# vsergeev/luaradio

Hardware: AMD Instinct MI355X
Metric: MSamples/s per block (128-tap complex FIR headline) + WBFM chain end-to-end (higher is better)
Workload: dtype f32

## Files before the change

### luaradio_amd/csrc/kernels_channelizer.h

```cpp
#pragma once
#include "common.h"
#include "kernels_fir.h"

#ifndef LRHIP_CHAN_EXP
#define LRHIP_CHAN_EXP 0
#endif

namespace lrhip {

#ifndef LRHIP_CHAN_INTERLEAVE
#define LRHIP_CHAN_INTERLEAVE 1
#endif
#ifndef LRHIP_CHAN_RT
#define LRHIP_CHAN_RT 1
#endif
#ifndef LRHIP_CHAN_KSLAB
#define LRHIP_CHAN_KSLAB 32
#endif
constexpr int CHAN_RT = LRHIP_CHAN_RT;
constexpr int CHAN_MT = 64 * CHAN_RT;
constexpr int CHAN_KSLAB = LRHIP_CHAN_KSLAB;

template <int NCT>
__global__ __launch_bounds__(256, CHAN_RT == 1 ? 2 : 1) void channelizer_kernel(const float *__restrict__ hist, const float *__restrict__ x,
                                                             const float *__restrict__ W, float *__restrict__ y,
                                                             int M, long n, long nframes, long first)
{
    constexpr int K2 = 16 * NCT;
    constexpr int K = K2 / 2;
    constexpr int DROW = K2 + 2;
    constexpr int WROW = K2 + 16;
    extern __shared__ __attribute__((aligned(16))) float lds[];
    const int tid = threadIdx.x, lane = tid & 63, wave = tid >> 6;
    const int col = lane & 15, kq = lane >> 4;
    const long f0 = (long)blockIdx.x * CHAN_MT;
    const int nsamp = (CHAN_MT - 1) * K + M;
    const int nflt = 2 * nsamp;
    float *ldsD = lds;
    const int dsize = ((nflt + 2 * (nflt / K2) + 2 + 3) / 4) * 4;
    float *ldsW = lds + dsize;

    const long p0 = first + f0 * K;
    const long xlo = p0 - (M - 1);
    if (xlo >= 0 && xlo + nsamp <= n && ((reinterpret_cast<uintptr_t>(x + 2 * xlo) & 15) == 0)) {
        const float4 *src = reinterpret_cast<const float4 *>(x + 2 * xlo);
        for (int i4 = tid; i4 < nflt / 4; i4 += 256) {
            float4 v = src[i4];
            int a = 4 * i4, p = a + 2 * (a / K2);
            *reinterpret_cast<float2 *>(ldsD + p) = make_float2(v.x, v.y);
            *reinterpret_cast<float2 *>(ldsD + p + 2) = make_float2(v.z, v.w);
        }
        for (int a = (nflt / 4) * 4 + tid; a < nflt; a += 256) ldsD[a + 2 * (a / K2)] = x[2 * xlo + a];
    } else {
        for (int r = tid; r < nsamp; r += 256) {
            int a = 2 * r, p = a + 2 * (a / K2);
            ldsD[p] = stream_at<2>(hist, x, p0 + r, 0, M, n);
            ldsD[p + 1] = stream_at<2>(hist, x, p0 + r, 1, M, n);
        }
    }

    constexpr int SLAB_F4 = CHAN_KSLAB * K2 / 4;
    constexpr int UW = (SLAB_F4 + 255) / 256;
    const float4 *W4 = reinterpret_cast<const float4 *>(W);
    static_assert(UW <= 8, "W slab prefetch: at most 8 float4 per thread");
    float4 w0, w1, w2, w3, w4, w5, w6, w7;
#define LR_CHAN_FOR8(OP) OP(0) OP(1) OP(2) OP(3) OP(4) OP(5) OP(6) OP(7)
#define LR_CHAN_LOAD(U)                                                                          \
    if (U < UW) {                                                                                \
        int i4 = tid + U * 256;                                                                  \
        w##U = W4[wbase + (i4 < SLAB_F4 ? i4 : SLAB_F4 - 1)];                                    \
    }
#define LR_CHAN_PUT(U)                                                                           \
    if (U < UW) {                                                                                \
        int i4 = tid + U * 256;                                                                  \
        if (i4 < SLAB_F4) *reinterpret_cast<float4 *>(wdst + ((4 * i4) / K2) * WROW + (4 * i4) % K2) = w##U; \
    }
    {
        const size_t wbase = 0;
        float *wdst = ldsW;
        LR_CHAN_FOR8(LR_CHAN_LOAD)
        LR_CHAN_FOR8(LR_CHAN_PUT)
    }
    __syncthreads();

    f32x4 acc[CHAN_RT][NCT];
#pragma unroll
    for (int r = 0; r < CHAN_RT; r++)
#pragma unroll
        for (int c = 0; c < NCT; c++) acc[r][c] = (f32x4){0.f, 0.f, 0.f, 0.f};
    const float *abase = ldsD + DROW * (wave * 16 * CHAN_RT + col) + kq;
    const int nslabs = 2 * M / CHAN_KSLAB;
    for (int s = 0; s < nslabs; s++) {
        const float *wcur = ldsW + (s & 1) * (CHAN_KSLAB * WROW);
#if LRHIP_CHAN_EXP == 1
        const bool more = false;
#else
        const bool more = s + 1 < nslabs;
#endif
        if (more) {
            const size_t wbase = (size_t)(s + 1) * SLAB_F4;
            LR_CHAN_FOR8(LR_CHAN_LOAD)
        }
        const float *ap = abase + CHAN_KSLAB * s + 2 * ((CHAN_KSLAB * s) / K2);
        const float *bp = wcur + kq * WROW + col;
        constexpr int NST = CHAN_KSLAB / 4;
        float av[2][CHAN_RT], bv[2][NCT];
        auto fetch = [&](int buf, int st) {
#pragma unroll
            for (int r = 0; r < CHAN_RT; r++) av[buf][r] = ap[16 * r * DROW + 4 * st];
#pragma unroll
            for (int c = 0; c < NCT; c++) bv[buf][c] = bp[4 * st * WROW + 16 * c];
        };
        fetch(0, 0);
#pragma unroll
        for (int st = 0; st < NST; st++) {
#if LRHIP_CHAN_INTERLEAVE
            if (st + 1 < NST) fetch((st + 1) & 1, st + 1);
#pragma unroll
            for (int c = 0; c < NCT; c++)
#pragma unroll
                for (int r = 0; r < CHAN_RT; r++)
                    acc[r][c] = __builtin_amdgcn_mfma_f32_16x16x4f32(av[st & 1][r], bv[st & 1][c], acc[r][c], 0, 0, 0);
#pragma unroll
            for (int i = 0; i < NCT * CHAN_RT; i++) {
                __builtin_amdgcn_sched_group_barrier(0x008, 1, 0);
                __builtin_amdgcn_sched_group_barrier(0x100, 1, 0);
            }
            __builtin_amdgcn_sched_barrier(0);
#else
            if (st + 1 < NST) fetch((st + 1) & 1, st + 1);
            __builtin_amdgcn_sched_barrier(0);
#pragma unroll
            for (int c = 0; c < NCT; c++)
#pragma unroll
                for (int r = 0; r < CHAN_RT; r++)
                    acc[r][c] = __builtin_amdgcn_mfma_f32_16x16x4f32(av[st & 1][r], bv[st & 1][c], acc[r][c], 0, 0, 0);
            __builtin_amdgcn_sched_barrier(0);
#endif
        }
        if (more) {
            float *wdst = ldsW + ((s + 1) & 1) * (CHAN_KSLAB * WROW);
            LR_CHAN_FOR8(LR_CHAN_PUT)
        }
#if LRHIP_CHAN_EXP != 1
        __syncthreads();
#endif
    }

#pragma unroll
    for (int rt = 0; rt < CHAN_RT; rt++)
#pragma unroll
        for (int c = 0; c < NCT; c++)
#pragma unroll
            for (int r = 0; r < 4; r++) {
                long f = f0 + (wave * CHAN_RT + rt) * 16 + 4 * kq + r;
                if (f < nframes) y[f * K2 + 16 * c + col] = acc[rt][c][r];
            }
}

#undef LR_CHAN_FOR8
#undef LR_CHAN_LOAD
#undef LR_CHAN_PUT

}
```

### luaradio_amd/csrc/stage_pfb.h

```cpp
#pragma once

struct PfbChannelizerStage : lrhip_stage {
    int seek(unsigned long long, unsigned long long *) override { return set_error("seek: not supported by the channelizer stage"); }
    long memory() const override { return -1; }
    int M = 0, K = 0, log2k = 0, P = 0, R = 1, D = 0;
    DeviceBuf taps, tw, hist[2];
    int cur = 0;
    unsigned long index = 0;
    unsigned phase = 0;
    const char *kind() const override { return "pfb_channelizer"; }
    unsigned long max_output(unsigned long n) const override { return (n / D + 1) * K; }
    static const char *refusal(unsigned ntaps, unsigned nchannels)
    {
        if (nchannels < 8 || nchannels > 4096 || (nchannels & (nchannels - 1))) return "pfb_channelizer: nchannels must be a power of two in [8, 4096]";
        const unsigned hi = 64 * nchannels < 65536 ? 64 * nchannels : 65536;
        if (ntaps < nchannels || ntaps > hi) return "pfb_channelizer: ntaps must be in [nchannels, min(64 * nchannels, 65536)]";
        return nullptr;
    }
    static const char *refusal(unsigned ntaps, unsigned nchannels, unsigned oversample)
    {
        if (oversample != 1 && oversample != 2 && oversample != 4) return "pfb_channelizer: oversample must be 1, 2 or 4";
        return refusal(ntaps, nchannels);
    }
    int frames_per_tile() const { return K <= 256 ? PFB_TILE_SMALL / K : K == 512 ? 8 : K == 1024 ? 4 : PFB_TILE_LARGE / K; }
    int frames_per_group() const { return K <= 1024 ? frames_per_tile() : PFB_SCRATCH / K; }
    int reset() override
    {
        cur = 0; index = 0; phase = 0;
        size_t hb = (size_t)(M - 1) * 2 * sizeof(float);
        return (zero_fill(hist[0], hb) || zero_fill(hist[1], hb)) ? -1 : 0;
    }
    template <int F, int NT>
    int launch(const float *x, long n, float *y, long nframes)
    {
        const int T = frames_per_tile(), G = frames_per_group();
        size_t lds_bytes = ((size_t)(T + G) * K + K / 2) * sizeof(float2);
        auto kern = pfb_channelizer_kernel<F, NT>;
        if (kernel_allow_lds(kern, lds_bytes)) return -1;
        unsigned grid = (unsigned)((nframes + T - 1) / T);
        hipLaunchKernelGGL(kern, dim3(grid), dim3(NT), lds_bytes, ctx().stream, (const float *)hist[cur].p, x, (const float *)taps.p,
                           (const float2 *)tw.p, y, M, log2k, P, T, G, n, nframes, (long)index);
        LR_LAUNCH_CHECK();
        return 0;
    }
    template <int RR, int F, int NT>
    int launch_oversampled(int T, int G, const float *x, long n, float *y, long nframes)
    {
        if (F > 1 && T % (RR * F)) return set_error("pfb_channelizer: a tile of %d frames does not hold blocks of %d frames in %d classes", T, F, RR);
        size_t lds_bytes = ((size_t)(T + G) * K + K / 2) * sizeof(float2);
        auto kern = pfb_oversampled_kernel<RR, F, NT>;
        if (kernel_allow_lds(kern, lds_bytes)) return -1;
        unsigned grid = (unsigned)((nframes + T - 1) / T);
        hipLaunchKernelGGL(kern, dim3(grid), dim3(NT), lds_bytes, ctx().stream, (const float *)hist[cur].p, x, (const float *)taps.p,
                           (const float2 *)tw.p, y, M, log2k, P, T, G, n, nframes, (long)index, (int)phase);
        LR_LAUNCH_CHECK();
        return 0;
    }
    int launch_oversampled_by_k(const float *x, long n, float *y, long nframes)
    {
        const int Ts = PFB_TILE_SMALL / K;
        if (R == 2) switch (log2k) {
            case 7: return launch_oversampled<2, 8, 256>(16, 16, x, n, y, nframes);
            case 8: return launch_oversampled<2, 4, 256>(8, 8, x, n, y, nframes);
            case 9: return launch_oversampled<2, 4, 1024>(8, 8, x, n, y, nframes);
            case 10: return launch_oversampled<2, 2, 512>(4, 4, x, n, y, nframes);
            case 11: return launch_oversampled<2, 4, 1024>(8, 1, x, n, y, nframes);
            case 12: return launch_oversampled<2, 1, 1024>(2, 1, x, n, y, nframes);
            default: return launch_oversampled<2, 8, 256>(Ts, Ts, x, n, y, nframes);
        }
        switch (log2k) {
            case 7: return launch_oversampled<4, 4, 256>(16, 16, x, n, y, nframes);
            case 8: return launch_oversampled<4, 2, 256>(8, 8, x, n, y, nframes);
            case 9: return launch_oversampled<4, 4, 1024>(16, 4, x, n, y, nframes);
            case 10: return launch_oversampled<4, 2, 512>(8, 1, x, n, y, nframes);
            case 11: return launch_oversampled<4, 2, 1024>(8, 1, x, n, y, nframes);
            case 12: return launch_oversampled<4, 1, 1024>(2, 1, x, n, y, nframes);
            default: return launch_oversampled<4, 8, 256>(Ts, Ts, x, n, y, nframes);
        }
    }
    long run(const void *in_dev, unsigned long n_in, void *out_dev, unsigned long cap) override
    {
        long n = (long)n_in;
        if (n <= 0) return 0;
        long nframes = n_in > index ? (long)((n_in - index + D - 1) / D) : 0;
        if ((unsigned long)(nframes * K) > cap) return set_error("pfb_channelizer: output capacity %lu < %ld", cap, nframes * K);
        const float *x = (const float *)in_dev;
        if (nframes > 0) {
            float *y = (float *)out_dev;
            int rc = R > 1 ? launch_oversampled_by_k(x, n, y, nframes)
                   : K <= 256 ? launch<8, 256>(x, n, y, nframes) : K == 512 ? launch<8, 1024>(x, n, y, nframes) : K == 1024 ? launch<4, 512>(x, n, y, nframes)
                   : K == 2048 ? launch<4, 1024>(x, n, y, nframes) : launch<2, 1024>(x, n, y, nframes);
            if (rc) return rc;
        }
        unsigned grid = grid_for((unsigned long)(M - 1) * 2, 256);
        hipLaunchKernelGGL(fir_history_kernel<2>, dim3(grid), dim3(256), 0, ctx().stream, (const float *)hist[cur].p, x, (float *)hist[cur ^ 1].p, M, n);
        LR_LAUNCH_CHECK();
        cur ^= 1;
        index = index + (unsigned long)nframes * D - n_in;
        phase = (unsigned)((phase + nframes) % R);
        return nframes * K;
    }
};

static ChannelizerStage *channelizer_build(const float *taps, unsigned ntaps, unsigned nchannels)
{
    auto q = new_stage<ChannelizerStage>();
    if (!q) return nullptr;
    int M = (int)ntaps, K = (int)nchannels, K2 = 2 * K;
    q->M = M; q->K = K;
    q->in_size = q->out_size = 8;
    std::vector<float> W((size_t)2 * M * K2);
    const double PI2 = 6.283185307179586476925286766559;
    for (int i = 0; i < M; i++)
        for (int c = 0; c < K; c++) {
            int j = M - 1 - i;
            double a = PI2 * (double)(((long)c * j) % K) / K, h = taps[j];
            float gr = (float)(h * std::cos(a)), gi = (float)(h * std::sin(a));
            W[(size_t)(2 * i) * K2 + 2 * c] = gr;
            W[(size_t)(2 * i + 1) * K2 + 2 * c] = -gi;
            W[(size_t)(2 * i) * K2 + 2 * c + 1] = gi;
            W[(size_t)(2 * i + 1) * K2 + 2 * c + 1] = gr;
        }
    if (upload(q->W, W.data(), W.size() * sizeof(float))) return nullptr;
    if (q->reset()) return nullptr;
    return q.release();
}
```

### luaradio_amd/csrc/stage_resample.h

```cpp
#pragma once

struct ResampleStage : lrhip_stage {
    int S = 2, M = 0, L = 1, HQ = 0;
    unsigned long D = 1;
    float c = 1.f;
    DeviceBuf d_taps, d_ttab, hist[2];
    int cur = 0;
    uint64_t Q0 = 0, m0 = 0;
    int interp_J = 0;
    static bool rational_supported(int L, unsigned long D) { return (L == 3 && D == 2) || (L == 2 && D == 3) || (L == 4 && D == 3) || (L == 3 && D == 4) || (L == 5 && D == 4) || (L == 4 && D == 5); }
    static int resample_rounds(long ntiles, long slots)
    {
        static const char *e = getenv("LRHIP_RESAMPLE_ROUNDS");
        if (e) return atoi(e) < 0 ? 0 : atoi(e);
        return persistent_rounds(ntiles, slots, 1);
    }
    static constexpr int SPAN_MAX = 6144;
    const char *kind() const override { return "resample"; }
    unsigned long max_output(unsigned long n) const override { return (n * (unsigned long)L) / D + 2; }
    int seek(unsigned long long n0, unsigned long long *n0_out) override
    {
        if (reset()) return -1;
        Q0 = n0;
        m0 = (n0 * (uint64_t)L + D - 1) / D;
        *n0_out = m0;
        return 0;
    }
    long memory() const override { return HQ; }
    void rate(unsigned long *num, unsigned long *den) const override { *num = D; *den = (unsigned long)L; }
    static bool fits(int M, int L, unsigned long D) { return L >= 1 && 256 * D / (unsigned long)L + (unsigned long)((M - 1) / L) + 4 <= (unsigned long)SPAN_MAX; }
    int reset() override
    {
        cur = 0; Q0 = 0; m0 = 0;
        size_t hb = (size_t)(HQ > 0 ? HQ : 1) * S * sizeof(float);
        return (zero_fill(hist[0], hb) || zero_fill(hist[1], hb)) ? -1 : 0;
    }
    long run(const void *in_dev, unsigned long n, void *out_dev, unsigned long cap) override
    {
        if (!n) return 0;
        uint64_t hi = (Q0 + n) * (uint64_t)L;
        uint64_t m_end = (hi + D - 1) / D;
        long n_out = (long)(m_end - m0);
        if ((unsigned long)n_out > cap) return set_error("resample: output capacity %lu < %ld", cap, n_out);
        const float *h = (const float *)hist[cur].p;
        float *ho = (float *)hist[cur ^ 1].p;
        if (interp_J > 0 && D == 1 && ((uintptr_t)in_dev & 7) == 0 && ((uintptr_t)out_dev & 7) == 0) {
            auto gi = [&](auto kern, size_t lds_bytes, int tq) -> int {
                const long ntiles = ((long)n + tq - 1) / tq, slots = chip_slots(kern, FIP_NT, lds_bytes);
                if (slots < 0) return -1;
                const int rounds = resample_rounds(ntiles, slots);
                hipLaunchKernelGGL(kern, dim3(persistent_grid(ntiles, slots, rounds)), dim3(FIP_NT), lds_bytes, ctx().stream, h, (const float *)in_dev, (const float *)d_ttab.p,
                                   (float *)out_dev, (long)n, HQ, c, ho, ablation_bits("LRHIP_INTERP_DBG"), rounds);
                return 0;
            };
#define LR_INTERP(LL, JJ) gi(fir_interp_kernel<LL, JJ>, (size_t)FipGeom<LL, JJ>::LDS_FLOATS * sizeof(float), FipGeom<LL, JJ>::TQ)
            int rc = L == 2 ? LR_INTERP(2, 64) : L == 3 ? LR_INTERP(3, 43) : L == 4 ? LR_INTERP(4, 32) : LR_INTERP(5, 26);
#undef LR_INTERP
            if (rc) return rc;
            LR_LAUNCH_CHECK();
            cur ^= 1;
            Q0 += n;
            m0 = m_end;
            return n_out;
        }
        static const bool no_rational = getenv("LRHIP_NO_RATIONAL_WIN") != nullptr;
        if (!no_rational && interp_J > 0 && D > 1 && ((uintptr_t)in_dev & 7) == 0 && ((uintptr_t)out_dev & 7) == 0) {
            auto gr = [&](auto kern, size_t lds_bytes, int tq) -> int {
                const long ntiles = ((long)n + (long)(Q0 % D) + tq - 1) / tq, slots = chip_slots(kern, 256, lds_bytes);
                if (slots < 0) return -1;
                const int rounds = resample_rounds(ntiles, slots);
                hipLaunchKernelGGL(kern, dim3(persistent_grid(ntiles, slots, rounds)), dim3(256), lds_bytes, ctx().stream, h, (const float *)in_dev, (const float *)d_ttab.p,
                                   (float *)out_dev, (long)n, n_out, m0, Q0, HQ, c, ho, rounds);
                return 0;
            };
#define LR_RAT(LL, DD, JJ, RR) gr(fir_rational_kernel<LL, DD, JJ, RR>, (size_t)FrrGeom<LL, DD, JJ, RR>::LDS_FLOATS * sizeof(float), FrrGeom<LL, DD, JJ, RR>::TQ)
            int rc = (L == 3 && D == 2) ? LR_RAT(3, 2, 43, 6) : (L == 2 && D == 3) ? LR_RAT(2, 3, 64, 9) : (L == 4 && D == 3) ? LR_RAT(4, 3, 32, 6)
                   : (L == 3 && D == 4) ? LR_RAT(3, 4, 43, 8) : (L == 5 && D == 4) ? LR_RAT(5, 4, 26, 8) : LR_RAT(4, 5, 32, 10);
#undef LR_RAT
            if (rc) return rc;
            LR_LAUNCH_CHECK();
            cur ^= 1;
            Q0 += n;
            m0 = m_end;
            return n_out;
        }
        int span_cap = (int)(256 * D / (unsigned long)L) + (M - 1) / L + 4;
        size_t lds_bytes = ((size_t)((((M - 1) / L + 1) * L + 3) & ~3) + (size_t)span_cap * S) * sizeof(float);
        auto go = [&](auto kern) -> int {
            if (kernel_allow_lds(kern, lds_bytes)) return -1;
            unsigned grid = n_out > 0 ? (unsigned)((n_out + 255) / 256) : 1;
            hipLaunchKernelGGL(kern, dim3(grid), dim3(256), lds_bytes, ctx().stream, h, (const float *)in_dev, (const float *)d_taps.p, (float *)out_dev, M, L,
                               (long)D, (long)n, n_out, m0, Q0, HQ, c, span_cap, ho);
            return 0;
        };
        int rc = S == 2 ? go(fir_resample_kernel<2>) : go(fir_resample_kernel<1>);
        if (rc) return rc;
        LR_LAUNCH_CHECK();
        cur ^= 1;
        Q0 += n;
        m0 = m_end;
        return n_out;
    }
};

struct ChannelizerStage : lrhip_stage {
    int seek(unsigned long long, unsigned long long *) override { return set_error("seek: not supported by the channelizer stage"); }
    long memory() const override { return -1; }
    int M = 0, K = 0;
    DeviceBuf W, hist[2];
    int cur = 0;
    unsigned long index = 0;
    const char *kind() const override { return "channelizer"; }
    unsigned long max_output(unsigned long n) const override { return (n / K + 1) * K; }
    int reset() override
    {
        cur = 0; index = 0;
        size_t hb = (size_t)(M - 1) * 2 * sizeof(float);
        return (zero_fill(hist[0], hb) || zero_fill(hist[1], hb)) ? -1 : 0;
    }
    template <int NCT>
    int launch(const float *x, long n, float *y, long nframes)
    {
        constexpr int K2 = 16 * NCT;
        int nflt = 2 * ((CHAN_MT - 1) * K + M);
        size_t dsize = (size_t)((nflt + 2 * (nflt / K2) + 2 + 3) / 4) * 4;
        size_t lds_bytes = (dsize + (size_t)2 * CHAN_KSLAB * (K2 + 16)) * sizeof(float);
        auto kern = channelizer_kernel<NCT>;
        if (kernel_allow_lds(kern, lds_bytes)) return -1;
        unsigned grid = (unsigned)((nframes + CHAN_MT - 1) / CHAN_MT);
        hipLaunchKernelGGL(kern, dim3(grid), dim3(256), lds_bytes, ctx().stream, (const float *)hist[cur].p, x, (const float *)W.p, y, M, n,
                           nframes, (long)index);
        LR_LAUNCH_CHECK();
        return 0;
    }
    long run(const void *in_dev, unsigned long n_in, void *out_dev, unsigned long cap) override
    {
        long n = (long)n_in;
        if (n <= 0) return 0;
        long nframes = n_in > index ? (long)((n_in - index + K - 1) / K) : 0;
        if ((unsigned long)(nframes * K) > cap) return set_error("channelizer: output capacity %lu < %ld", cap, nframes * K);
        const float *x = (const float *)in_dev;
        if (nframes > 0) {
            int rc = K == 32 ? launch<4>(x, n, (float *)out_dev, nframes) : launch<8>(x, n, (float *)out_dev, nframes);
            if (rc) return rc;
        }
        unsigned grid = grid_for((unsigned long)(M - 1) * 2, 256);
        hipLaunchKernelGGL(fir_history_kernel<2>, dim3(grid), dim3(256), 0, ctx().stream, (const float *)hist[cur].p, x, (float *)hist[cur ^ 1].p, M, n);
        LR_LAUNCH_CHECK();
        cur ^= 1;
        index = index + (unsigned long)nframes * K - n_in;
        return nframes * K;
    }
};
```

Baseline: 328,700.

## Exploit real-tap DFT symmetry in channelizer with split re/im planes

Replaces the complex-as-2x2-real weight matrix with a real-valued cos/sin weight matrix covering only half the channels. Input is deinterleaved into separate real and imaginary LDS planes, and the output bins are reconstructed as conjugate-symmetric pairs from the re/im accumulators. This roughly halves the weight matrix size and its LDS traffic, and cuts the MFMA count per frame. The cost is a more complex epilogue with special handling for bins 0 and K/2. It also removes the RT and KSLAB tuning knobs.

After: 316,500. 0.963x the previous value.

```diff
diff --git a/luaradio_amd/csrc/kernels_channelizer.h b/luaradio_amd/csrc/kernels_channelizer.h
--- a/luaradio_amd/csrc/kernels_channelizer.h
+++ b/luaradio_amd/csrc/kernels_channelizer.h
@@ -1,44 +1,40 @@
 #pragma once
 #include "common.h"
 #include "kernels_fir.h"
-
-#ifndef LRHIP_CHAN_EXP
-#define LRHIP_CHAN_EXP 0
-#endif
 
 namespace lrhip {
 
 #ifndef LRHIP_CHAN_INTERLEAVE
 #define LRHIP_CHAN_INTERLEAVE 1
 #endif
-#ifndef LRHIP_CHAN_RT
-#define LRHIP_CHAN_RT 1
-#endif
-#ifndef LRHIP_CHAN_KSLAB
-#define LRHIP_CHAN_KSLAB 32
-#endif
-constexpr int CHAN_RT = LRHIP_CHAN_RT;
-constexpr int CHAN_MT = 64 * CHAN_RT;
-constexpr int CHAN_KSLAB = LRHIP_CHAN_KSLAB;
+constexpr int CHAN_MT = 64;
+constexpr int CHAN_KSLAB = 32;
+
+__host__ __device__ constexpr int chan_plane_floats(int M, int K)
+{
+    int nsamp = (CHAN_MT - 1) * K + M;
+    return ((nsamp + 2 * (nsamp / K) + 2 + 3) / 4) * 4;
+}
+__host__ __device__ constexpr int chan_lds_floats(int M, int K) { return 2 * chan_plane_floats(M, K) + 2 * CHAN_KSLAB * (K + 16); }
 
 template <int NCT>
-__global__ __launch_bounds__(256, CHAN_RT == 1 ? 2 : 1) void channelizer_kernel(const float *__restrict__ hist, const float *__restrict__ x,
+__global__ __launch_bounds__(256, 2) void channelizer_kernel(const float *__restrict__ hist, const float *__restrict__ x,
                                                              const float *__restrict__ W, float *__restrict__ y,
                                                              int M, long n, long nframes, long first)
 {
-    constexpr int K2 = 16 * NCT;
-    constexpr int K = K2 / 2;
-    constexpr int DROW = K2 + 2;
-    constexpr int WROW = K2 + 16;
+    constexpr int K = 16 * NCT;
+    constexpr int NH = NCT / 2;
+    constexpr int DROW = K + 2;
+    constexpr int WROW = K + 16;
     extern __shared__ __attribute__((aligned(16))) float lds[];
     const int tid = threadIdx.x, lane = tid & 63, wave = tid >> 6;
     const int col = lane & 15, kq = lane >> 4;
     const long f0 = (long)blockIdx.x * CHAN_MT;
     const int nsamp = (CHAN_MT - 1) * K + M;
     const int nflt = 2 * nsamp;
-    float *ldsD = lds;
-    const int dsize = ((nflt + 2 * (nflt / K2) + 2 + 3) / 4) * 4;
-    float *ldsW = lds + dsize;
+    float *ldsRe = lds;
+    float *ldsIm = lds + chan_plane_floats(M, K);
+    float *ldsW = ldsIm + chan_plane_floats(M, K);
 
     const long p0 = first + f0 * K;
     const long xlo = p0 - (M - 1);
@@ -46,25 +42,28 @@
         const float4 *src = reinterpret_cast<const float4 *>(x + 2 * xlo);
         for (int i4 = tid; i4 < nflt / 4; i4 += 256) {
             float4 v = src[i4];
-            int a = 4 * i4, p = a + 2 * (a / K2);
-            *reinterpret_cast<float2 *>(ldsD + p) = make_float2(v.x, v.y);
-            *reinterpret_cast<float2 *>(ldsD + p + 2) = make_float2(v.z, v.w);
+            int r = 2 * i4, p = r + 2 * (r / K);
+            *reinterpret_cast<float2 *>(ldsRe + p) = make_float2(v.x, v.z);
+            *reinterpret_cast<float2 *>(ldsIm + p) = make_float2(v.y, v.w);
         }
-        for (int a = (nflt / 4) * 4 + tid; a < nflt; a += 256) ldsD[a + 2 * (a / K2)] = x[2 * xlo + a];
+        for (int a = (nflt / 4) * 4 + tid; a < nflt; a += 256) {
+            int r = a >> 1;
+            ((a & 1) ? ldsIm : ldsRe)[r + 2 * (r / K)] = x[2 * xlo + a];
+        }
     } else {
         for (int r = tid; r < nsamp; r += 256) {
-            int a = 2 * r, p = a + 2 * (a / K2);
-            ldsD[p] = stream_at<2>(hist, x, p0 + r, 0, M, n);
-            ldsD[p + 1] = stream_at<2>(hist, x, p0 + r, 1, M, n);
+            int p = r + 2 * (r / K);
+            ldsRe[p] = stream_at<2>(hist, x, p0 + r, 0, M, n);
+            ldsIm[p] = stream_at<2>(hist, x, p0 + r, 1, M, n);
         }
     }
 
-    constexpr int SLAB_F4 = CHAN_KSLAB * K2 / 4;
+    constexpr int SLAB_F4 = CHAN_KSLAB * K / 4;
     constexpr int UW = (SLAB_F4 + 255) / 256;
     const float4 *W4 = reinterpret_cast<const float4 *>(W);
-    static_assert(UW <= 8, "W slab prefetch: at most 8 float4 per thread");
-    float4 w0, w1, w2, w3, w4, w5, w6, w7;
-#define LR_CHAN_FOR8(OP) OP(0) OP(1) OP(2) OP(3) OP(4) OP(5) OP(6) OP(7)
+    static_assert(UW <= 2, "Wp slab prefetch: at most 2 float4 per thread");
+    float4 w0, w1;
+#define LR_CHAN_FOR2(OP) OP(0) OP(1)
 #define LR_CHAN_LOAD(U)                                                                          \
     if (U < UW) {                                                                                \
         int i4 = tid + U * 256;                                                                  \
@@ -73,92 +72,87 @@
 #define LR_CHAN_PUT(U)                                                                           \
     if (U < UW) {                                                                                \
         int i4 = tid + U * 256;                                                                  \
-        if (i4 < SLAB_F4) *reinterpret_cast<float4 *>(wdst + ((4 * i4) / K2) * WROW + (4 * i4) % K2) = w##U; \
+        if (i4 < SLAB_F4) *reinterpret_cast<float4 *>(wdst + ((4 * i4) / K) * WROW + (4 * i4) % K) = w##U; \
     }
     {
         const size_t wbase = 0;
         float *wdst = ldsW;
-        LR_CHAN_FOR8(LR_CHAN_LOAD)
-        LR_CHAN_FOR8(LR_CHAN_PUT)
+        LR_CHAN_FOR2(LR_CHAN_LOAD)
+        LR_CHAN_FOR2(LR_CHAN_PUT)
     }
     __syncthreads();
 
-    f32x4 acc[CHAN_RT][NCT];
+    f32x4 acc_re[NCT], acc_im[NCT];
 #pragma unroll
-    for (int r = 0; r < CHAN_RT; r++)
-#pragma unroll
-        for (int c = 0; c < NCT; c++) acc[r][c] = (f32x4){0.f, 0.f, 0.f, 0.f};
-    const float *abase = ldsD + DROW * (wave * 16 * CHAN_RT + col) + kq;
-    const int nslabs = 2 * M / CHAN_KSLAB;
+    for (int c = 0; c < NCT; c++) acc_re[c] = acc_im[c] = (f32x4){0.f, 0.f, 0.f, 0.f};
+    const int aoff = DROW * (wave * 16 + col) + kq;
+    const int nslabs = M / CHAN_KSLAB;
     for (int s = 0; s < nslabs; s++) {
         const float *wcur = ldsW + (s & 1) * (CHAN_KSLAB * WROW);
-#if LRHIP_CHAN_EXP == 1
-        const bool more = false;
-#else
         const bool more = s + 1 < nslabs;
-#endif
         if (more) {
             const size_t wbase = (size_t)(s + 1) * SLAB_F4;
-            LR_CHAN_FOR8(LR_CHAN_LOAD)
+            LR_CHAN_FOR2(LR_CHAN_LOAD)
         }
-        const float *ap = abase + CHAN_KSLAB * s + 2 * ((CHAN_KSLAB * s) / K2);
+        const int koff = aoff + CHAN_KSLAB * s + 2 * ((CHAN_KSLAB * s) / K);
+        const float *apr = ldsRe + koff, *api = ldsIm + koff;
         const float *bp = wcur + kq * WROW + col;
         constexpr int NST = CHAN_KSLAB / 4;
-        float av[2][CHAN_RT], bv[2][NCT];
+        float ar[2], ai[2], bv[2][NCT];
         auto fetch = [&](int buf, int st) {
-#pragma unroll
-            for (int r = 0; r < CHAN_RT; r++) av[buf][r] = ap[16 * r * DROW + 4 * st];
+            ar[buf] = apr[4 * st];
+            ai[buf] = api[4 * st];
 #pragma unroll
             for (int c = 0; c < NCT; c++) bv[buf][c] = bp[4 * st * WROW + 16 * c];
         };
         fetch(0, 0);
 #pragma unroll
         for (int st = 0; st < NST; st++) {
+            if (st + 1 < NST) fetch((st + 1) & 1, st + 1);
+#if !LRHIP_CHAN_INTERLEAVE
+            __builtin_amdgcn_sched_barrier(0);
+#endif
+#pragma unroll
+            for (int c = 0; c < NCT; c++) {
+                acc_re[c] = __builtin_amdgcn_mfma_f32_16x16x4f32(ar[st & 1], bv[st & 1][c], acc_re[c], 0, 0, 0);
+                acc_im[c] = __builtin_amdgcn_mfma_f32_16x16x4f32(ai[st & 1], bv[st & 1][c], acc_im[c], 0, 0, 0);
+            }
 #if LRHIP_CHAN_INTERLEAVE
-            if (st + 1 < NST) fetch((st + 1) & 1, st + 1);
 #pragma unroll
-            for (int c = 0; c < NCT; c++)
-#pragma unroll
-                for (int r = 0; r < CHAN_RT; r++)
-                    acc[r][c] = __builtin_amdgcn_mfma_f32_16x16x4f32(av[st & 1][r], bv[st & 1][c], acc[r][c], 0, 0, 0);
-#pragma unroll
-            for (int i = 0; i < NCT * CHAN_RT; i++) {
+            for (int i = 0; i < 2 * NCT; i++) {
                 __builtin_amdgcn_sched_group_barrier(0x008, 1, 0);
                 __builtin_amdgcn_sched_group_barrier(0x100, 1, 0);
             }
+#endif
             __builtin_amdgcn_sched_barrier(0);
-#else
-            if (st + 1 < NST) fetch((st + 1) & 1, st + 1);
-            __builtin_amdgcn_sched_barrier(0);
-#pragma unroll
-            for (int c = 0; c < NCT; c++)
-#pragma unroll
-                for (int r = 0; r < CHAN_RT; r++)
-                    acc[r][c] = __builtin_amdgcn_mfma_f32_16x16x4f32(av[st & 1][r], bv[st & 1][c], acc[r][c], 0, 0, 0);
-            __builtin_amdgcn_sched_barrier(0);
-#endif
         }
         if (more) {
             float *wdst = ldsW + ((s + 1) & 1) * (CHAN_KSLAB * WROW);
-            LR_CHAN_FOR8(LR_CHAN_PUT)
+            LR_CHAN_FOR2(LR_CHAN_PUT)
         }
-#if LRHIP_CHAN_EXP != 1
         __syncthreads();
-#endif
     }
 
+    float2 *y2 = reinterpret_cast<float2 *>(y);
 #pragma unroll
-    for (int rt = 0; rt < CHAN_RT; rt++)
+    for (int t = 0; t < NH; t++)
 #pragma unroll
-        for (int c = 0; c < NCT; c++)
-#pragma unroll
-            for (int r = 0; r < 4; r++) {
-                long f = f0 + (wave * CHAN_RT + rt) * 16 + 4 * kq + r;
-                if (f < nframes) y[f * K2 + 16 * c + col] = acc[rt][c][r];
+        for (int r = 0; r < 4; r++) {
+            const long f = f0 + wave * 16 + 4 * kq + r;
+            if (f >= nframes) continue;
+            const int c = 16 * t + col;
+            const float p1 = acc_re[t][r], p4 = acc_im[t][r], q1 = acc_re[t + NH][r], q4 = acc_im[t + NH][r];
+            if (c == 0) {
+                y2[f * K] = make_float2(p1 + 0.f * p4, p4 + 0.f * p1);
+                y2[f * K + K / 2] = make_float2(q1 + 0.f * q4, q4 + 0.f * q1);
+            } else {
+                y2[f * K + c] = make_float2(p1 - q4, q1 + p4);
+                y2[f * K + K - c] = make_float2(p1 + q4, p4 - q1);
             }
+        }
 }
 
-#undef LR_CHAN_FOR8
+#undef LR_CHAN_FOR2
 #undef LR_CHAN_LOAD
 #undef LR_CHAN_PUT
 
diff --git a/luaradio_amd/csrc/stage_pfb.h b/luaradio_amd/csrc/stage_pfb.h
--- a/luaradio_amd/csrc/stage_pfb.h
+++ b/luaradio_amd/csrc/stage_pfb.h
@@ -106,20 +106,17 @@
 {
     auto q = new_stage<ChannelizerStage>();
     if (!q) return nullptr;
-    int M = (int)ntaps, K = (int)nchannels, K2 = 2 * K;
+    int M = (int)ntaps, K = (int)nchannels, H = K / 2;
     q->M = M; q->K = K;
     q->in_size = q->out_size = 8;
-    std::vector<float> W((size_t)2 * M * K2);
+    std::vector<float> W((size_t)M * K);
     const double PI2 = 6.283185307179586476925286766559;
     for (int i = 0; i < M; i++)
-        for (int c = 0; c < K; c++) {
+        for (int c = 0; c < H; c++) {
             int j = M - 1 - i;
             double a = PI2 * (double)(((long)c * j) % K) / K, h = taps[j];
-            float gr = (float)(h * std::cos(a)), gi = (float)(h * std::sin(a));
-            W[(size_t)(2 * i) * K2 + 2 * c] = gr;
-            W[(size_t)(2 * i + 1) * K2 + 2 * c] = -gi;
-            W[(size_t)(2 * i) * K2 + 2 * c + 1] = gi;
-            W[(size_t)(2 * i + 1) * K2 + 2 * c + 1] = gr;
+            W[(size_t)i * K + c] = (float)(h * std::cos(a));
+            W[(size_t)i * K + H + c] = c ? (float)(h * std::sin(a)) : (float)((j & 1) ? -h : h);
         }
     if (upload(q->W, W.data(), W.size() * sizeof(float))) return nullptr;
     if (q->reset()) return nullptr;
diff --git a/luaradio_amd/csrc/stage_resample.h b/luaradio_amd/csrc/stage_resample.h
--- a/luaradio_amd/csrc/stage_resample.h
+++ b/luaradio_amd/csrc/stage_resample.h
@@ -121,10 +121,7 @@
     template <int NCT>
     int launch(const float *x, long n, float *y, long nframes)
     {
-        constexpr int K2 = 16 * NCT;
-        int nflt = 2 * ((CHAN_MT - 1) * K + M);
-        size_t dsize = (size_t)((nflt + 2 * (nflt / K2) + 2 + 3) / 4) * 4;
-        size_t lds_bytes = (dsize + (size_t)2 * CHAN_KSLAB * (K2 + 16)) * sizeof(float);
+        size_t lds_bytes = (size_t)chan_lds_floats(M, 16 * NCT) * sizeof(float);
         auto kern = channelizer_kernel<NCT>;
         if (kernel_allow_lds(kern, lds_bytes)) return -1;
         unsigned grid = (unsigned)((nframes + CHAN_MT - 1) / CHAN_MT);
@@ -141,7 +138,7 @@
         if ((unsigned long)(nframes * K) > cap) return set_error("channelizer: output capacity %lu < %ld", cap, nframes * K);
         const float *x = (const float *)in_dev;
         if (nframes > 0) {
-            int rc = K == 32 ? launch<4>(x, n, (float *)out_dev, nframes) : launch<8>(x, n, (float *)out_dev, nframes);
+            int rc = K == 32 ? launch<2>(x, n, (float *)out_dev, nframes) : launch<4>(x, n, (float *)out_dev, nframes);
             if (rc) return rc;
         }
         unsigned grid = grid_for((unsigned long)(M - 1) * 2, 256);
```
